# marc345/Dense2Sparse-ViT

Measured on AMD Instinct MI355X. Metric: training images/s, DeiT-S 224 keep_ratio=0.5 (dense-to-sparse ViT train step, teacher fwd + student fwd/bwd + AdamW), higher is better.
Workload: dtype f32; 1 GPU; DeiT-Small 224x224 patch16, 1-stage prune keep_ratio=0.5 @ block 3 (196->98 tokens), large LN predictor, kl_div mask loss, per-GPU batch 128; global_batch=128, parallelism=dp1

## Files before the change

dense2sparse-vit_amd/csrc/gemm_common.h:

```cpp
#pragma once
#include "d2s_common.h"

namespace d2s_gemm {

enum Epi : int {
    EPI_NONE = 0,
    EPI_BIAS = 1,
    EPI_BIAS_RELU = 2,
    EPI_BIAS_GELU = 3,
    EPI_BIAS_RESID = 4,
    EPI_MUL_GELU_GRAD = 5,
    EPI_MUL_RELU_MASK = 6,
    EPI_BIAS_ROWADD = 7,
    EPI_ACCUM = 8,
    EPI_BIAS_GELU_Z16 = 9,
    EPI_MUL_GELU_GRAD_Z16 = 10,
    EPI_BIAS_RESID_ROWSCALE = 11,
};

struct GemmArgs {
    const float* A; const float* B; float* C;
    const float* bias; const float* aux; float* aux_out;
    long lda, ldb, ldc, ldaux;
    int M, N, K;
    int epi;
    int k_per_slice;
    long slab_stride;
    int aux_rows;
    int vecA, vecB;
    int remap_rows_per_img; int remap_skip;
    int stagger;
    int vec_epilogue;
    float* colsum;
    int colsum_accumulate;
    const void* a16; void* c16;
    const void* b16;
    int aux_bf16;
    const float* rowscale; int rows_per_group;
};

typedef __bf16 bf16x4_epi __attribute__((ext_vector_type(4)));

template <int EPI, int MT, int NT>
__device__ __forceinline__ void store_tile_out(const GemmArgs& p, float* __restrict__ Cb, const f32x16 (&acc)[MT][NT], int mbase,
                                               int nbase, int half) {
#pragma unroll
    for (int nt = 0; nt < NT; ++nt) {
        const int n = nbase + nt * 32;
        if (n >= p.N) continue;
        float bias = 0.f;
        if (EPI == EPI_BIAS || EPI == EPI_BIAS_RELU || EPI == EPI_BIAS_GELU || EPI == EPI_BIAS_RESID || EPI == EPI_BIAS_ROWADD ||
            EPI == EPI_BIAS_RESID_ROWSCALE)
            bias = p.bias ? p.bias[n] : 0.f;
#pragma unroll
        for (int mt = 0; mt < MT; ++mt) {
#pragma unroll
            for (int r = 0; r < 16; ++r) {
                const int m = mbase + mt * 32 + mfma32_row(r, half);
                if (m >= p.M) continue;
                float v = acc[mt][nt][r];
                long orow = m;
                if (EPI == EPI_BIAS_ROWADD && p.remap_rows_per_img > 0)
                    orow = (long)m + (long)(m / p.remap_rows_per_img) * p.remap_skip + p.remap_skip;
                float* cp = Cb + orow * p.ldc + n;
                if (EPI == EPI_BIAS) v += bias;
                if (EPI == EPI_BIAS_RELU) v = fmaxf(v + bias, 0.f);
                if (EPI == EPI_BIAS_GELU) {
                    v += bias;
                    if (p.aux_out && p.aux_bf16) reinterpret_cast<__bf16*>(p.aux_out)[(long)m * p.ldc + n] = (__bf16)v;
                    else if (p.aux_out) p.aux_out[(long)m * p.ldc + n] = v;
                    v = gelu_erf(v);
                }
                if (EPI == EPI_BIAS_RESID) v += bias + p.aux[(long)m * p.ldaux + n];
                if (EPI == EPI_BIAS_RESID_ROWSCALE) {
                    const float s = p.rowscale[m / p.rows_per_group];
                    v = s == 0.f ? p.aux[(long)m * p.ldaux + n] : s * (v + bias) + p.aux[(long)m * p.ldaux + n];
                }
                if (EPI == EPI_MUL_GELU_GRAD)
                    v *= gelu_erf_grad(p.aux_bf16 ? (float)reinterpret_cast<const __bf16*>(p.aux)[(long)m * p.ldaux + n] : p.aux[(long)m * p.ldaux + n]);
                if (EPI == EPI_MUL_RELU_MASK) v = p.aux[(long)m * p.ldaux + n] > 0.f ? v : 0.f;
                if (EPI == EPI_BIAS_ROWADD) v += bias + p.aux[(long)(m % p.aux_rows) * p.ldaux + n];
                if (EPI == EPI_ACCUM) v += *cp;
                *cp = v;
            }
        }
    }
}

__host__ __device__ constexpr int epi_stage_floats(int NT) { return 16 * (NT * 32 + 4); }

template <int EPI, int MT, int NT, bool C16 = false>
// ... 125 lines not shown
```

dense2sparse-vit_amd/csrc/gemm_f32.hip:

```cpp
#include "gemm_common.h"

namespace {
using namespace d2s_gemm;

constexpr int BK = 16;

#ifdef D2S_STAMPS
__device__ unsigned long long g_stamps_f32[8 * 65536];
#define FSTAMP(i) if (threadIdx.x == 0 && blockIdx.x < 65536 && blockIdx.z == 0) g_stamps_f32[8 * blockIdx.x + (i)] = __builtin_amdgcn_s_memrealtime()
#define FSTAMPC(i) if (threadIdx.x == 0 && blockIdx.x < 65536 && blockIdx.z == 0) g_stamps_f32[8 * blockIdx.x + (i)] = __builtin_amdgcn_s_memtime()
#define FSTAMPID(i) if (threadIdx.x == 0 && blockIdx.x < 65536 && blockIdx.z == 0) g_stamps_f32[8 * blockIdx.x + (i)] = \
    ((unsigned long long)__builtin_amdgcn_s_getreg((15 << 11) | (0 << 6) | 4)) | ((unsigned long long)__builtin_amdgcn_s_getreg((3 << 11) | (0 << 6) | 20) << 32)
#else
#define FSTAMP(i)
#define FSTAMPC(i)
#define FSTAMPID(i)
#endif

template <int LAY, int BR>
__device__ __forceinline__ void load_tile(const float* __restrict__ P, long ld, int row0, int k0, int rows, int kend,
                                          int vec, int tid, f32x4 (&r)[BR / 64]) {
#pragma unroll
    for (int i = 0; i < BR / 64; ++i) {
        const int f = tid + i * 256;
// ... 196 lines not shown
        f32x4 t = csum[0];
#pragma unroll
        for (int i = 1; i < BM / 64; ++i) t += csum[i];
        *reinterpret_cast<f32x4*>(&smem[(tid / CH) * BM + (tid % CH) * 4]) = t;
        __syncthreads();
        if (tid < BM && row0 + tid < p.M) {
            float s = 0.f;
#pragma unroll
            for (int g = 0; g < G; ++g) s += smem[g * BM + tid];
            float* o = p.colsum + (long)blockIdx.z * p.M + row0 + tid;
            *o = (gridDim.z == 1 && p.colsum_accumulate) ? *o + s : s;
        }
        __syncthreads();
    }

    FSTAMP(2); FSTAMPC(5);
    float* Cb = p.C + (long)blockIdx.z * p.slab_stride;
    const int epi = (gridDim.z > 1) ? (int)EPI_NONE : p.epi;
    static_assert(4 * epi_stage_floats(NT) <= 2 * BK * (BM + BN), "epilogue staging must fit the operand buffers");
    if (p.vec_epilogue) {
        store_tile_dispatch_lds<MT, NT>(epi, p, Cb, acc, row0 + wm * WM, col0 + wn * WN, lane, smem + wave * epi_stage_floats(NT));
#ifdef D2S_STAMPS
        __builtin_amdgcn_s_waitcnt(0);
        FSTAMP(3);
#endif
        return;
    }
    const int mbase = row0 + wm * WM, nbase = col0 + wn * WN + l31;
    switch (epi) {
        case EPI_BIAS: store_tile_out<EPI_BIAS, MT, NT>(p, Cb, acc, mbase, nbase, half); break;
        case EPI_BIAS_RELU: store_tile_out<EPI_BIAS_RELU, MT, NT>(p, Cb, acc, mbase, nbase, half); break;
        case EPI_BIAS_GELU: store_tile_out<EPI_BIAS_GELU, MT, NT>(p, Cb, acc, mbase, nbase, half); break;
        case EPI_BIAS_RESID: store_tile_out<EPI_BIAS_RESID, MT, NT>(p, Cb, acc, mbase, nbase, half); break;
        case EPI_MUL_GELU_GRAD: store_tile_out<EPI_MUL_GELU_GRAD, MT, NT>(p, Cb, acc, mbase, nbase, half); break;
        case EPI_MUL_RELU_MASK: store_tile_out<EPI_MUL_RELU_MASK, MT, NT>(p, Cb, acc, mbase, nbase, half); break;
        case EPI_BIAS_ROWADD: store_tile_out<EPI_BIAS_ROWADD, MT, NT>(p, Cb, acc, mbase, nbase, half); break;
        case EPI_ACCUM: store_tile_out<EPI_ACCUM, MT, NT>(p, Cb, acc, mbase, nbase, half); break;
        case EPI_BIAS_RESID_ROWSCALE: store_tile_out<EPI_BIAS_RESID_ROWSCALE, MT, NT>(p, Cb, acc, mbase, nbase, half); break;
        default: store_tile_out<EPI_NONE, MT, NT>(p, Cb, acc, mbase, nbase, half); break;
    }
}

template <int BR>
__device__ __forceinline__ void store_tile_rk(float* __restrict__ S, int tid, const f32x4 (&r)[BR / 64]) {
#pragma unroll
    for (int i = 0; i < BR / 64; ++i) {
        const int f = tid + i * 256;
        const int row = f >> 2, kq = f & 3;
        *reinterpret_cast<f32x4*>(&S[row * BK + ((kq ^ ((row >> 2) & 3)) << 2)]) = r[i];
    }
}

template <int BLAY, int BM, int BN>
__global__ __launch_bounds__(256, (BM == 128 && BN == 128) ? 3 : 1) void gemm_f32_rk_kernel(GemmArgs p) {
    constexpr int WM = BM / 2, WN = BN / 2, MT = WM / 32, NT = WN / 32;
    __shared__ __attribute__((aligned(16))) float smem[2 * BK * (BM + BN)];
    float* As = smem;
    float* Bs = smem + 2 * BK * BM;
    const int tid = threadIdx.x, lane = tid & 63, wave = tid >> 6;
    const int half = lane >> 5, l31 = lane & 31;
    const int wm = wave >> 1, wn = wave & 1;
    const int nbm = (p.M + BM - 1) / BM, nbn = (p.N + BN - 1) / BN;
    const int nwg = nbm * nbn;
    int bid = blockIdx.x;
    {
        const int q = nwg >> 3, r = nwg & 7, xcd = bid & 7, idx = bid >> 3;
        bid = (xcd < r ? xcd * (q + 1) : r * (q + 1) + (xcd - r) * q) + idx;
    }
    const int bm = bid / nbn, bn = bid % nbn;
    const int row0 = bm * BM, col0 = bn * BN;
    const int kbeg = blockIdx.z * p.k_per_slice;
    const int kend = min(p.K, kbeg + p.k_per_slice);
    const int nk = (kend - kbeg + BK - 1) / BK;

    f32x16 acc[MT][NT];
#pragma unroll
    for (int i = 0; i < MT; ++i)
#pragma unroll
        for (int j = 0; j < NT; ++j)
#pragma unroll
            for (int r = 0; r < 16; ++r) acc[i][j][r] = 0.f;

    f32x4 ra[BM / 64], rb[BN / 64];
    long offa[BM / 64], offb[BN / 64];
    tile_offsets<0, BM>(p.lda, row0, p.M, tid, offa);
    tile_offsets<BLAY, BN>(p.ldb, col0, p.N, tid, offb);
    if (nk > 0) {
        load_tile_fast<0, BM>(p.A, p.lda, kbeg, offa, ra);
        load_tile_fast<BLAY, BN>(p.B, p.ldb, kbeg, offb, rb);
        store_tile_rk<BM>(As, tid, ra);
        if (BLAY == 0) store_tile_rk<BN>(Bs, tid, rb);
        else store_tile<1, BN>(Bs, tid, rb);
    }
    __syncthreads();

    int a_off[MT][2], b_off[NT][2];
#pragma unroll
    for (int i = 0; i < MT; ++i) {
        const int row = wm * WM + i * 32 + l31;
#pragma unroll
        for (int c = 0; c < 2; ++c) a_off[i][c] = row * BK + (((2 * half + c) ^ ((row >> 2) & 3)) << 2);
    }
#pragma unroll
    for (int j = 0; j < NT; ++j) {
        const int row = wn * WN + j * 32 + l31;
#pragma unroll
        for (int c = 0; c < 2; ++c) b_off[j][c] = row * BK + (((2 * half + c) ^ ((row >> 2) & 3)) << 2);
    }

    for (int kt = 0; kt < nk; ++kt) {
        const int cur = kt & 1;
        const int kn = kbeg + min(kt + 1, nk - 1) * BK;
        load_tile_fast<0, BM>(p.A, p.lda, kn, offa, ra);
        load_tile_fast<BLAY, BN>(p.B, p.ldb, kn, offb, rb);
        const float* Ac = As + cur * BK * BM;
        const float* Bc = Bs + cur * BK * BN;
        f32x4 av[MT][2], bv[NT][2];
#pragma unroll
        for (int c = 0; c < 2; ++c) {
#pragma unroll
            for (int i = 0; i < MT; ++i) av[i][c] = *reinterpret_cast<const f32x4*>(Ac + a_off[i][c]);
            if (BLAY == 0) {
#pragma unroll
                for (int j = 0; j < NT; ++j) bv[j][c] = *reinterpret_cast<const f32x4*>(Bc + b_off[j][c]);
            }
        }
#pragma unroll
        for (int s = 0; s < 8; ++s) {
            float bs[NT];
            if (BLAY == 0) {
#pragma unroll
                for (int j = 0; j < NT; ++j) bs[j] = bv[j][s >> 2][s & 3];
            } else {
                const int k = 8 * half + s;
                const int sw = (((k >> 2) & 3) << 3) ^ ((k & 1) << 4);
#pragma unroll
                for (int j = 0; j < NT; ++j) bs[j] = Bc[k * BN + ((wn * WN + j * 32 + l31) ^ sw)];
            }
#pragma unroll
            for (int i = 0; i < MT; ++i)
#pragma unroll
                for (int j = 0; j < NT; ++j) acc[i][j] = mfma32(av[i][s >> 2][s & 3], bs[j], acc[i][j]);
        }
        if (kt + 1 < nk) {
            store_tile_rk<BM>(As + (cur ^ 1) * BK * BM, tid, ra);
            if (BLAY == 0) store_tile_rk<BN>(Bs + (cur ^ 1) * BK * BN, tid, rb);
            else store_tile<1, BN>(Bs + (cur ^ 1) * BK * BN, tid, rb);
        }
        __syncthreads();
    }

    float* Cb = p.C + (long)blockIdx.z * p.slab_stride;
    const int epi = (gridDim.z > 1) ? (int)EPI_NONE : p.epi;
    store_tile_dispatch_lds<MT, NT>(epi, p, Cb, acc, row0 + wm * WM, col0 + wn * WN, lane, smem + wave * epi_stage_floats(NT));
}

__global__ __launch_bounds__(256) void splitk_reduce_kernel(const float* __restrict__ ws, float* __restrict__ C,
                                                            long ldc, int M, int N, int slabs, long slab_stride,
                                                            int accumulate, const float* __restrict__ colsum_ws,
                                                            float* __restrict__ colsum_out) {
    const long idx = (long)blockIdx.x * 256 + threadIdx.x;
    const long total = (long)M * N;
    if (idx >= total) {
        const long m = idx - total;
        if (colsum_out && m < M) {
            float s = 0.f;
            for (int z = 0; z < slabs; ++z) s += colsum_ws[(long)z * M + m];
            colsum_out[m] = accumulate ? colsum_out[m] + s : s;
        }
        return;
    }
    const int m = (int)(idx / N), n = (int)(idx % N);
    float s = 0.f;
    for (int z = 0; z < slabs; ++z) s += ws[(long)z * slab_stride + (long)m * N + n];
    float* cp = C + (long)m * ldc + n;
    *cp = accumulate ? (*cp + s) : s;
}

__global__ __launch_bounds__(256) void splitk_reduce_vec_kernel(const float* __restrict__ ws, float* __restrict__ C, long ldc, int M, int N,
                                                                int slabs, long slab_stride, int accumulate,
                                                                const float* __restrict__ colsum_ws, float* __restrict__ colsum_out) {
    const long idx = (long)blockIdx.x * 256 + threadIdx.x;
    const int nq = N >> 2;
    const long total = (long)M * nq;
    if (idx >= total) {
        const long m = idx - total;
        if (colsum_out && m < M) {
            float s = 0.f;
            for (int z = 0; z < slabs; ++z) s += colsum_ws[(long)z * M + m];
            colsum_out[m] = accumulate ? colsum_out[m] + s : s;
        }
        return;
    }
    const int m = (int)(idx / nq), n = (int)(idx % nq) * 4;
    const float* src = ws + (long)m * N + n;
    f32x4 s = {0.f, 0.f, 0.f, 0.f};
    for (int z = 0; z < slabs; ++z) {
        const f32x4 v = *reinterpret_cast<const f32x4*>(src + (long)z * slab_stride);
#pragma unroll
        for (int j = 0; j < 4; ++j) s[j] += v[j];
    }
    f32x4* cp = reinterpret_cast<f32x4*>(C + (long)m * ldc + n);
    if (accumulate) {
        const f32x4 o = *cp;
#pragma unroll
        for (int j = 0; j < 4; ++j) s[j] += o[j];
    }
// ... 88 lines not shown
#pragma unroll
    for (int i = 0; i < 4; ++i) {
        const int f = tid + i * 256, c = f >> 4, r4 = (f & 15) * 4;
        if (c0 + c < C) {
#pragma unroll
            for (int j = 0; j < 4; ++j)
                if (r0 + r4 + j < R) dst[(long)(c0 + c) * R + r0 + r4 + j] = t[r4 + j][c];
        }
    }
}

__global__ __launch_bounds__(256) void colsum_partial_kernel(const float* __restrict__ X, long ldx, int M, int N,
                                                             int rows_per_slice, float* __restrict__ part) {
    __shared__ float red[4][64];
    const int lane = threadIdx.x & 63, wave = threadIdx.x >> 6;
    const int n = blockIdx.x * 64 + lane;
    const int m0 = blockIdx.y * rows_per_slice, m1 = min(M, m0 + rows_per_slice);
    float s = 0.f;
    if (n < N)
        for (int m = m0 + wave; m < m1; m += 4) s += X[(long)m * ldx + n];
    red[wave][lane] = s;
    __syncthreads();
    if (wave == 0 && n < N) part[(long)blockIdx.y * N + n] = red[0][lane] + red[1][lane] + red[2][lane] + red[3][lane];
}
__global__ __launch_bounds__(1024) void colsum_fold_wide_kernel(const float* __restrict__ part, int N, int slices, float* __restrict__ out,
                                                                int accumulate) {
    __shared__ float red[64][17];
    const int col = threadIdx.x & 15, kl = threadIdx.x >> 4;
    const int n = blockIdx.x * 16 + col;
    float s = 0.f;
    if (n < N)
        for (int z = kl; z < slices; z += 64) s += part[(long)z * N + n];
    red[kl][col] = s;
    __syncthreads();
    if (kl == 0 && n < N) {
        float t = 0.f;
#pragma unroll 8
        for (int k = 0; k < 64; ++k) t += red[k][col];
        out[n] = accumulate ? out[n] + t : t;
    }
}

__global__ __launch_bounds__(256) void colsum_final_kernel(const float* __restrict__ part, int N, int slices,
                                                           float* __restrict__ out, int accumulate) {
    const int n = blockIdx.x * 256 + threadIdx.x;
    if (n >= N) return;
    float s = 0.f;
    for (int z = 0; z < slices; ++z) s += part[(long)z * N + n];
    out[n] = accumulate ? out[n] + s : s;
}


struct Tile { int bm, bn; float penalty; };
inline Tile pick_tile(int M, int N) {
    const Tile cand[4] = {{128, 128, 1.00f}, {128, 64, 1.04f}, {64, 128, 1.05f}, {64, 64, 1.10f}};
    Tile best = cand[0];
    float best_cost = 1e30f;
    for (const Tile& t : cand) {
        const long nwg = (long)((M + t.bm - 1) / t.bm) * ((N + t.bn - 1) / t.bn);
        const long per_cu = (nwg + 255) / 256;
        const float pipe = per_cu >= 3 ? 1.0f : per_cu == 2 ? 0.85f : 0.6f;
        const float cost = (float)per_cu * t.bm * t.bn * t.penalty / pipe;
        if (cost < best_cost) { best_cost = cost; best = t; }
    }
    return best;
}

template <int ALAY, int BLAY, bool FAST>
inline void launch_gemm_f(const Tile& t, dim3 grid, hipStream_t stream, const GemmArgs& p) {
    dim3 block(256);
    if (t.bm == 128 && t.bn == 128) hipLaunchKernelGGL((gemm_f32_kernel<ALAY, BLAY, 128, 128, FAST>), grid, block, 0, stream, p);
    else if (t.bm == 128) hipLaunchKernelGGL((gemm_f32_kernel<ALAY, BLAY, 128, 64, FAST>), grid, block, 0, stream, p);
    else if (t.bn == 128) hipLaunchKernelGGL((gemm_f32_kernel<ALAY, BLAY, 64, 128, FAST>), grid, block, 0, stream, p);
    else hipLaunchKernelGGL((gemm_f32_kernel<ALAY, BLAY, 64, 64, FAST>), grid, block, 0, stream, p);
}
template <int BLAY>
inline void launch_gemm_rk(const Tile& t, dim3 grid, hipStream_t stream, const GemmArgs& p) {
    dim3 block(256);
    if (t.bm == 128 && t.bn == 128) hipLaunchKernelGGL((gemm_f32_rk_kernel<BLAY, 128, 128>), grid, block, 0, stream, p);
    else if (t.bm == 128) hipLaunchKernelGGL((gemm_f32_rk_kernel<BLAY, 128, 64>), grid, block, 0, stream, p);
    else if (t.bn == 128) hipLaunchKernelGGL((gemm_f32_rk_kernel<BLAY, 64, 128>), grid, block, 0, stream, p);
    else hipLaunchKernelGGL((gemm_f32_rk_kernel<BLAY, 64, 64>), grid, block, 0, stream, p);
}
template <int ALAY, int BLAY>
inline void launch_gemm(const Tile& t, dim3 grid, hipStream_t stream, const GemmArgs& p, bool fast) {
    if (fast && p.vec_epilogue && ALAY == 0) launch_gemm_rk<BLAY>(t, grid, stream, p);
    else if (fast) launch_gemm_f<ALAY, BLAY, true>(t, grid, stream, p);
    else launch_gemm_f<ALAY, BLAY, false>(t, grid, stream, p);
}

}

namespace d2s_gemm {
size_t split_workspace_bytes(int split, int M, int N, int K);
int launch_split_gemm(const GemmArgs& p, int b_cols, int split, void* workspace, size_t workspace_bytes, hipStream_t stream);
size_t split_tn_pieces_bytes(int split, int M, int N, int K);
int split_tn_colsum_partials(int K);
bool split_tn_use_dma(int M, int N, int K);
int split_tn_dma_slices(int M, int N, int K);
int launch_split_gemm_tn(const GemmArgs& p, int split, int slices, void* pieces_ws, float* colsum_part, hipStream_t stream, int* colsum_parts);
}
static int splitk_target() {
    static const int t = [] {
        int dev = 0, cus = 0;
        if (hipGetDevice(&dev) != hipSuccess || hipDeviceGetAttribute(&cus, hipDeviceAttributeMultiprocessorCount, dev) != hipSuccess || cus <= 0)
            cus = 256;
        return 3 * cus;
    }();
    return t;
}
static inline size_t ws_align(size_t x) { return (x + 255) & ~(size_t)255; }
extern "C" size_t d2s_colsum_workspace_bytes(int M, int N);
extern "C" int d2s_colsum_f32(const float* X, long ldx, int M, int N, float* out, int accumulate, void* workspace,
                              size_t workspace_bytes, hipStream_t stream);
static int nt_slices(int tiles, int K) {
    if (K < 512 || tiles > 512) return 1;
    int best = 1;
    float best_cost = 1e30f;
    const int smax = K / 256 < 8 ? K / 256 : 8;
    for (int sl = 1; sl <= smax; ++sl) {
        const long per_cu = ((long)tiles * sl + 255) / 256;
        const float pipe = per_cu >= 3 ? 1.0f : per_cu == 2 ? 0.85f : 0.6f;
        const float cost = (float)per_cu / ((float)sl * pipe) + 0.04f * (sl - 1);
        if (cost < best_cost - 1e-6f) { best_cost = cost; best = sl; }
    }
    return best;
}
static int splitk_slices(int tiles, int K) {
    int slices = splitk_target() / tiles;
    const int max_slices = (K + 255) / 256;
    if (slices > max_slices) slices = max_slices;
    if (slices < 1) slices = 1;
    return slices;
}

#ifdef D2S_STAMPS
extern "C" int d2s_debug_read_stamps_f32(unsigned long long* host_out, int n_wg) {
    return hipMemcpyFromSymbol(host_out, HIP_SYMBOL(g_stamps_f32), (size_t)n_wg * 8 * sizeof(unsigned long long)) == hipSuccess ? 0 : -1;
}
#endif

extern "C" {

size_t d2s_gemm_f32_workspace_bytes(int layout, int M, int N, int K, int mode) {
    if (layout != 2 && mode != 0) return split_workspace_bytes(mode == 1 ? 3 : 1, M, N, K);
    if (layout != 2) {
        const Tile t = pick_tile(M, N);
        const int sl = nt_slices(((M + t.bm - 1) / t.bm) * ((N + t.bn - 1) / t.bn), K);
        return sl > 1 ? (size_t)sl * M * N * sizeof(float) : 0;
    }
    const int tiles = ((M + 127) / 128) * ((N + 127) / 128);
    if (mode != 2) {
        const int slices = splitk_slices(tiles, K);
        return slices <= 1 ? 0 : ((size_t)slices * M * N + (size_t)slices * M) * sizeof(float);
    }
    const int slices = split_tn_use_dma(M, N, K) ? split_tn_dma_slices(M, N, K) : splitk_slices(tiles, K);
    return ws_align(((size_t)(slices + 1) * M * N) * sizeof(float)) + ws_align(split_tn_pieces_bytes(1, M, N, K)) + (size_t)split_tn_colsum_partials(K) * M * sizeof(float);
}

static int gemm_impl(int layout, const float* A, long lda, const float* B, long ldb, float* C, long ldc, int M, int N,
                     int K, int epilogue, const float* bias, const float* aux, long ldaux, float* aux_out, int aux_rows,
                     int remap_rows_per_img, int remap_skip, int accumulate, void* workspace, size_t workspace_bytes,
                     hipStream_t stream, float* colsum_out, int mode, const void* a16 = nullptr, void* c16 = nullptr, const void* b16 = nullptr,
                     const float* rowscale = nullptr, int rows_per_group = 0) {
    if (b16 && (mode != 2 || (layout != 2 && (K % 32 != 0 || !aligned16(b16))) || (layout == 2 && (reinterpret_cast<uintptr_t>(b16) & 7)))) return D2S_ERR_ARG;
    if ((!A && !(a16 && layout != 2) && !(b16 && layout == 2)) || (!B && !(a16 && layout == 2) && !(b16 && layout != 2)) || (!C && !c16) || M <= 0 || N <= 0 || K <= 0 || layout < 0 || layout > 2 || mode < 0 || mode > 2) return D2S_ERR_ARG;
    if ((a16 || c16) && (mode != 2 || (layout != 2 && accumulate) || remap_rows_per_img > 0)) return D2S_ERR_ARG;
    if (layout == 2 && c16) return D2S_ERR_ARG;
    if (layout == 2 && a16) {
        if ((reinterpret_cast<uintptr_t>(a16) & 7) != 0) return D2S_ERR_ARG;
    }
    if ((a16 && layout != 2 && (K % 32 != 0 || !aligned16(a16))) || (c16 && (N % 32 != 0 || !aligned16(c16)))) return D2S_ERR_ARG;
    int aux_bf16 = 0;
    if (epilogue == EPI_BIAS_GELU_Z16 || epilogue == EPI_MUL_GELU_GRAD_Z16) {
        const float* z = epilogue == EPI_BIAS_GELU_Z16 ? aux_out : aux;
        if (mode != 2 || layout == 2 || !z || (reinterpret_cast<uintptr_t>(z) & 7) || N % 4 != 0 || (epilogue == EPI_MUL_GELU_GRAD_Z16 && ldaux % 4 != 0) ||
            (epilogue == EPI_BIAS_GELU_Z16 && ldc % 4 != 0))
            return D2S_ERR_ARG;
        aux_bf16 = 1;
        epilogue = epilogue == EPI_BIAS_GELU_Z16 ? EPI_BIAS_GELU : EPI_MUL_GELU_GRAD;
    }
    if (epilogue == EPI_BIAS_RESID_ROWSCALE) {
        if (!rowscale || rows_per_group <= 0 || layout == 2 || accumulate || !aux) return D2S_ERR_ARG;
    } else if (epilogue < EPI_NONE || epilogue > EPI_ACCUM) return D2S_ERR_ARG;
    if ((epilogue == EPI_BIAS_RESID || epilogue == EPI_MUL_GELU_GRAD || epilogue == EPI_MUL_RELU_MASK ||
         epilogue == EPI_BIAS_ROWADD) && !aux)
        return D2S_ERR_ARG;
    GemmArgs p;
    p.aux_bf16 = aux_bf16;
    p.A = A; p.B = B; p.C = C; p.bias = bias; p.aux = aux; p.aux_out = aux_out;
    p.lda = lda; p.ldb = ldb; p.ldc = ldc; p.ldaux = ldaux;
    p.M = M; p.N = N; p.K = K; p.epi = epilogue; p.aux_rows = aux_rows > 0 ? aux_rows : 1;
    p.remap_rows_per_img = remap_rows_per_img; p.remap_skip = remap_skip;
    p.colsum = nullptr; p.colsum_accumulate = accumulate;
    p.a16 = a16; p.c16 = c16; p.b16 = b16;
    p.rowscale = rowscale; p.rows_per_group = rows_per_group > 0 ? rows_per_group : 1;
    {
        p.stagger = 0;
        p.vec_epilogue = 0;
    }
    const int alay = layout == 2 ? 1 : 0, blay = layout == 0 ? 0 : 1;
    p.vecA = aligned16(A) && (lda % 4 == 0) && (alay == 0 ? (K % 4 == 0) : (M % 4 == 0));
    p.vecB = aligned16(B) && (ldb % 4 == 0) && (blay == 0 ? (K % 4 == 0) : (N % 4 == 0));
    if (mode != 0 && layout != 2) {
        if (accumulate) p.epi = EPI_ACCUM;
        p.k_per_slice = K;
        p.slab_stride = 0;
        return launch_split_gemm(p, layout == 1 ? 1 : 0, mode == 1 ? 3 : 1, workspace, workspace_bytes, stream);
    }
    if (layout == 2 && mode == 2) {
        const int tiles = ((M + 127) / 128) * ((N + 127) / 128);
        int slices = split_tn_use_dma(M, N, K) ? split_tn_dma_slices(M, N, K) : splitk_slices(tiles, K);
        const int Kp = ((K + 63) / 64) * 64;
        int kper = (((Kp + slices - 1) / slices + 63) / 64) * 64;
        slices = (Kp + kper - 1) / kper;
        const size_t slab_bytes = ws_align(((size_t)(slices + 1) * M * N) * sizeof(float));
        const size_t piece_bytes = ws_align(split_tn_pieces_bytes(1, M, N, K));
        const size_t cs_bytes = (size_t)split_tn_colsum_partials(K) * M * sizeof(float);
        if (!workspace || workspace_bytes < slab_bytes + piece_bytes + cs_bytes) return D2S_ERR_WORKSPACE;
        unsigned char* wsb = static_cast<unsigned char*>(workspace);
        p.k_per_slice = kper;
        p.epi = EPI_NONE;
        p.C = reinterpret_cast<float*>(wsb);
        p.ldc = N;
        p.slab_stride = (long)M * N;
        p.remap_rows_per_img = 0;
        float* cs_part = colsum_out ? reinterpret_cast<float*>(wsb + slab_bytes + piece_bytes) : nullptr;
        int cs_parts = 0;
        int rc = launch_split_gemm_tn(p, 1, slices, wsb + slab_bytes, cs_part, stream, &cs_parts);
        if (rc != D2S_OK) return rc;
        const long total = (long)M * N;
        hipLaunchKernelGGL(splitk_reduce_kernel, dim3((unsigned)((total + 255) / 256)), dim3(256), 0, stream,
                           reinterpret_cast<const float*>(wsb), C, ldc, M, N, slices, (long)M * N, accumulate,
                           static_cast<const float*>(nullptr), static_cast<float*>(nullptr));
        if (colsum_out)
            hipLaunchKernelGGL(colsum_fold_wide_kernel, dim3((M + 15) / 16), dim3(1024), 0, stream, cs_part, M, cs_parts,
                               colsum_out, accumulate);
        return d2s_check_launch();
    }
    Tile tile = layout == 2 ? Tile{128, 128, 1.f} : pick_tile(M, N);
    const int tiles = ((M + tile.bm - 1) / tile.bm) * ((N + tile.bn - 1) / tile.bn);
    int slices = layout == 2 ? splitk_slices(tiles, K) : nt_slices(tiles, K);
    int kper = (K + slices - 1) / slices;
    kper = ((kper + BK - 1) / BK) * BK;
    slices = (K + kper - 1) / kper;
    p.k_per_slice = kper;
    p.slab_stride = 0;
    float* realC = C;
    if (accumulate && layout != 2 && p.epi == EPI_NONE) p.epi = EPI_ACCUM;
    const GemmArgs real = p;
    if (slices > 1 && layout != 2) {
        const size_t need = (size_t)slices * M * N * sizeof(float);
        if (!workspace || workspace_bytes < need) return D2S_ERR_WORKSPACE;
        p.C = static_cast<float*>(workspace);
        p.ldc = N;
        p.slab_stride = (long)M * N;
        p.remap_rows_per_img = 0;
    } else if (slices > 1) {
        const size_t need = ((size_t)slices * M * N + (size_t)slices * M) * sizeof(float);
        if (!workspace || workspace_bytes < need) return D2S_ERR_WORKSPACE;
        p.C = static_cast<float*>(workspace);
        p.ldc = N;
        p.slab_stride = (long)M * N;
        p.remap_rows_per_img = 0;
        if (colsum_out) p.colsum = static_cast<float*>(workspace) + (size_t)slices * M * N;
    } else {
        if (accumulate) p.epi = EPI_ACCUM;
        p.colsum = colsum_out;
    }
    p.vec_epilogue = (epilogue_vec_ok(p) && (p.slab_stride % 4 == 0)) ? 1 : 0;
    dim3 grid(tiles, 1, slices), block(256);
    const bool fast = p.vecA && p.vecB && (K % BK == 0) && (alay == 0 || M >= 4) && (blay == 0 || N >= 4);
    if (layout == 0) launch_gemm<0, 0>(tile, grid, stream, p, fast);
    else if (layout == 1) launch_gemm<0, 1>(tile, grid, stream, p, fast);
    else launch_gemm<1, 1>(tile, grid, stream, p, fast);
    if (slices > 1 && layout != 2) {
        const long total = (long)M * N;
        hipLaunchKernelGGL(splitk_reduce_epi_kernel, dim3((unsigned)((total + 255) / 256)), block, 0, stream, real,
                           static_cast<const float*>(workspace), slices, (long)M * N);
    } else if (slices > 1) {
        if ((N % 4 == 0) && (ldc % 4 == 0) && aligned16(realC) && aligned16(workspace) && (((long)M * N) % 4 == 0)) {
            const long total = (long)M * (N / 4) + (colsum_out ? M : 0);
            hipLaunchKernelGGL(splitk_reduce_vec_kernel, dim3((unsigned)((total + 255) / 256)), block, 0, stream,
                               static_cast<const float*>(workspace), realC, ldc, M, N, slices, (long)M * N, accumulate, p.colsum, colsum_out);
        } else {
            const long total = (long)M * N + (colsum_out ? M : 0);
            hipLaunchKernelGGL(splitk_reduce_kernel, dim3((unsigned)((total + 255) / 256)), block, 0, stream,
                               static_cast<const float*>(workspace), realC, ldc, M, N, slices, (long)M * N, accumulate,
                               p.colsum, colsum_out);
        }
    }
    return d2s_check_launch();
}

int d2s_gemm_f32(int layout, const float* A, long lda, const float* B, long ldb, float* C, long ldc, int M, int N,
                 int K, int epilogue, const float* bias, const float* aux, long ldaux, float* aux_out, int aux_rows,
                 int remap_rows_per_img, int remap_skip, int accumulate, int mode, void* workspace, size_t workspace_bytes,
                 hipStream_t stream) {
    return gemm_impl(layout, A, lda, B, ldb, C, ldc, M, N, K, epilogue, bias, aux, ldaux, aux_out, aux_rows, remap_rows_per_img,
                     remap_skip, accumulate, workspace, workspace_bytes, stream, nullptr, mode);
}

int d2s_gemm_f32_bf16io(int layout, const float* A, long lda, const float* B, long ldb, float* C, long ldc, int M, int N, int K,
                        int epilogue, const float* bias, const float* aux, long ldaux, float* aux_out, const void* a_bf16, const void* b_bf16,
                        void* c_bf16, void* workspace, size_t workspace_bytes, hipStream_t stream) {
    if (layout == 2) return D2S_ERR_ARG;
    return gemm_impl(layout, A, lda, B, ldb, C, ldc, M, N, K, epilogue, bias, aux, ldaux, aux_out, 0, 0, 0, 0, workspace, workspace_bytes,
                     stream, nullptr, 2, a_bf16, c_bf16, b_bf16);
}

int d2s_gemm_f32_rowscale(int layout, const float* A, long lda, const float* B, long ldb, float* C, long ldc, int M, int N, int K,
                          const float* bias, const float* aux, long ldaux, const float* rowscale, int rows_per_group, int mode,
                          const void* a_bf16, const void* b_bf16, void* c_bf16, void* workspace, size_t workspace_bytes, hipStream_t stream) {
    if (layout == 2 || !rowscale || rows_per_group <= 0) return D2S_ERR_ARG;
    return gemm_impl(layout, A, lda, B, ldb, C, ldc, M, N, K, EPI_BIAS_RESID_ROWSCALE, bias, aux, ldaux, nullptr, 0, 0, 0, 0, workspace,
                     workspace_bytes, stream, nullptr, mode, a_bf16, c_bf16, b_bf16, rowscale, rows_per_group);
}

size_t d2s_linear_wgrad_workspace_bytes(int tokens, int n_out, int n_in, int mode) {
    return d2s_gemm_f32_workspace_bytes(2, n_out, n_in, tokens, mode);
}
int d2s_linear_wgrad_f32(const float* dy, long lddy, const float* x, long ldx, float* dW, long lddw, float* db, int tokens,
                         int n_out, int n_in, int accumulate, int mode, void* workspace, size_t workspace_bytes, hipStream_t stream) {
    return gemm_impl(2, dy, lddy, x, ldx, dW, lddw, n_out, n_in, tokens, EPI_NONE, nullptr, nullptr, 0, nullptr, 0, 0, 0,
                     accumulate, workspace, workspace_bytes, stream, db, mode);
}
int d2s_linear_wgrad_f32_bf16x(const float* dy, const void* dy_bf16, long lddy, const void* x_bf16, long ldx, float* dW, long lddw, float* db,
                               int tokens, int n_out, int n_in, int accumulate, void* workspace, size_t workspace_bytes, hipStream_t stream) {
    if (!x_bf16 || (!dy && !dy_bf16)) return D2S_ERR_ARG;
    return gemm_impl(2, dy, lddy, nullptr, ldx, dW, lddw, n_out, n_in, tokens, EPI_NONE, nullptr, nullptr, 0, nullptr, 0, 0, 0,
                     accumulate, workspace, workspace_bytes, stream, db, 2, x_bf16, nullptr, dy_bf16);
}

int d2s_transpose_f32(const float* src, float* dst, int R, int C, hipStream_t stream) {
    if (!src || !dst || R <= 0 || C <= 0) return D2S_ERR_ARG;
    hipLaunchKernelGGL(transpose_kernel, dim3((C + 63) / 64, (R + 63) / 64), dim3(256), 0, stream, src, dst, R, C);
    return d2s_check_launch();
}

int d2s_transpose_batched_f32(const float* src_base, float* dst_base, const void* tile_desc, int n_tiles, hipStream_t stream) {
    if (!src_base || !dst_base || !tile_desc || n_tiles <= 0) return D2S_ERR_ARG;
    static_assert(sizeof(TransposeTile) == 32, "descriptor layout is part of the C ABI");
    hipLaunchKernelGGL(transpose_batched_kernel, dim3(n_tiles), dim3(256), 0, stream, src_base, dst_base, static_cast<const TransposeTile*>(tile_desc));
    return d2s_check_launch();
}

size_t d2s_colsum_workspace_bytes(int M, int N) {
    int slices = (M + 511) / 512;
    if (slices > 128) slices = 128;
    if (slices < 1) slices = 1;
    return (size_t)slices * N * sizeof(float);
}

int d2s_colsum_f32(const float* X, long ldx, int M, int N, float* out, int accumulate, void* workspace,
                   size_t workspace_bytes, hipStream_t stream) {
// ... 15 lines not shown
```

dense2sparse-vit_amd/d2s/lib.py:

```python
import ctypes
import os

import torch

_HERE = os.path.dirname(os.path.abspath(__file__))
LIB_PATH = os.environ.get("D2S_LIB_PATH") or os.path.join(os.path.dirname(_HERE), "lib", "libd2s_hip.so")

P, I, L, F, Z = ctypes.c_void_p, ctypes.c_int, ctypes.c_long, ctypes.c_float, ctypes.c_size_t

_SIGS = {
    "d2s_gemm_f32_workspace_bytes": (Z, [I, I, I, I, I]),
    "d2s_gemm_f32": (I, [I, P, L, P, L, P, L, I, I, I, I, P, P, L, P, I, I, I, I, I, P, Z]),
    "d2s_gemm_f32_bf16io": (I, [I, P, L, P, L, P, L, I, I, I, I, P, P, L, P, P, P, P, P, Z]),
    "d2s_convert_bf16": (I, [P, P, L]),
    "d2s_linear_wgrad_workspace_bytes": (Z, [I, I, I, I]),
    "d2s_linear_wgrad_f32": (I, [P, L, P, L, P, L, P, I, I, I, I, I, P, Z]),
    "d2s_linear_wgrad_f32_bf16x": (I, [P, P, L, P, L, P, L, P, I, I, I, I, P, Z]),
    "d2s_batchnorm_workspace_bytes": (Z, [L, I]),
    "d2s_batchnorm_fwd": (I, [P, P, P, P, P, P, P, P, L, I, F, F, I, P, Z]),
    "d2s_batchnorm_bwd": (I, [P, P, P, P, P, P, P, P, I, I, I, L, I, P, Z]),
    "d2s_transpose_f32": (I, [P, P, I, I]),
    "d2s_transpose_batched_f32": (I, [P, P, P, I]),
    "d2s_colsum_workspace_bytes": (Z, [I, I]),
    "d2s_colsum_f32": (I, [P, L, I, I, P, I, P, Z]),
# ... 70 lines not shown
    "d2s_block_saved_floats": (L, [I, I, I, I, I, I]),
    "d2s_block_bwd_scratch_floats": (L, [I, I, I, I, I]),
    "d2s_block_workspace_bytes": (Z, [I, I, I, I, I]),
    "d2s_block_wgrad_workspace_bytes": (Z, [I, I, I, I, I]),
    "d2s_block_fwd_f32": (I, [P, P, I, I, I, I, I, F, F, P, P, P, I, I, P, Z]),
    "d2s_block_bwd_f32": (I, [P, P, P, P, P, I, I, I, I, I, F, P, P, P, I, P, Z, P, Z, P]),
    "d2s_drop_path_scales": (I, [P, P, I, I, ctypes.c_ulonglong]),
    "d2s_gemm_f32_rowscale": (I, [I, P, L, P, L, P, L, I, I, I, P, P, L, P, I, I, P, P, P, P, Z]),
    "d2s_scale_rows": (I, [P, P, P, L, I, I]),
    "d2s_drop_path_fwd": (I, [P, P, P, I, L]),
    "d2s_block_bwd_dp_scratch_floats": (L, [I, I, I, I, I]),
    "d2s_block_fwd_f32_dp": (I, [P, P, P, P, I, I, I, I, I, F, F, P, P, P, I, I, P, Z]),
    "d2s_block_bwd_f32_dp": (I, [P, P, P, P, P, P, P, I, I, I, I, I, F, P, P, P, I, P, Z, P, Z, P]),
    "d2s_adamw_chunk_elems": (I, None),
    "d2s_adamw_step": (I, [P, P, P, P, P, I, F, F, F, I, F, P]),
    "d2s_adamw_step_ema": (I, [P, P, P, P, P, I, F, F, F, I, F, P, P, F]),
    "d2s_adamw_step_clip": (I, [P, P, P, P, P, I, F, F, F, I, F, P, P, F, P]),
    "d2s_grad_accumulate": (I, [P, P, P, I, I]),
    "d2s_grad_clip_coef": (I, [P, P, I, F, F, P, P]),
    "d2s_augment_desc_ints": (I, None),
    "d2s_augment_images": (I, [P, L, P, I, I, I, I, I, I, ctypes.c_ulonglong, P, P]),
    "d2s_augment_labels": (I, [P, I, I, F, F, P]),
    "d2s_randaug_max_ops": (I, None),
    "d2s_randaug_op_ints": (I, None),
    "d2s_randaug_scratch_bytes": (Z, [I, I]),
    "d2s_randaug_apply": (I, [P, P, I, I, P, P]),
    "d2s_augment_ops_scratch_bytes": (Z, [I, I]),
    "d2s_augment_images_ops": (I, [P, L, P, P, I, I, I, I, I, I, ctypes.c_ulonglong, P, P, P]),
    "d2s_gumbel_noise": (I, [P, L, ctypes.c_ulonglong]),
    "d2s_gumbel_from_bits": (I, [P, P, L]),
    "d2s_gumbel_keep_fwd": (I, [P, P, P, P, P, P, P, L]),
    "d2s_gumbel_keep_bwd": (I, [P, P, P, P, P, P, L]),
    "d2s_policy_pool_fwd": (I, [P, P, P, P, P, I, I, I]),
    "d2s_policy_pool_bwd": (I, [P, P, P, P, P, P, P, P, I, I, I]),
    "d2s_ratio_rows_fwd": (I, [P, F, P, P, I, I]),
    "d2s_ratio_rows_bwd": (I, [P, P, F, P, I, I]),
}

_SIGS_EXT = {
    "d2s_attn_keyw_fwd_bf16": (I, [P, I, P, P, P, P, I, I, I, F]),
    "d2s_tome_match_bf16": (I, [P, I, I, I, I, P, P, P, P, P]),
}

_SIGS_SQUEEZE = {
    "d2s_squeeze_match": (I, [P, P, P, I, I, I, I, P, P]),
    "d2s_gather_squeeze_fwd": (I, [P, P, P, P, P, I, I, I, I, P, P]),
    "d2s_gather_squeeze_bwd": (I, [P, P, P, P, P, P, I, I, I, I, P]),
}

_SIGS_ATS = {
    "d2s_ats_select": (I, [P, P, I, P, P, I, I, I, I, I, I, P, P, P, P]),
}

_lib = None


class D2SError(RuntimeError):
    pass


def load():
    global _lib
    if _lib is not None:
        return _lib
    if not os.path.exists(LIB_PATH):
        raise D2SError(f"{LIB_PATH} not found - build it with `python -c 'import __graft_entry__ as g; g.build()'` "
                       "(or `make -C dense2sparse-vit_amd/csrc`). The d2s path has no CPU fallback.")
    lib = ctypes.CDLL(LIB_PATH)
    for name, (res, args) in list(_SIGS.items()) + list(_SIGS_EXT.items()) + list(_SIGS_SQUEEZE.items()) + list(_SIGS_ATS.items()):
        fn = getattr(lib, name)
        fn.restype = res
        fn.argtypes = [] if args is None else list(args) + ([P] if res is I else [])
    _lib = lib
    return lib


def exported_symbols():
    return sorted(_SIGS)


def extension_symbols():
    return sorted(_SIGS_EXT)


def squeeze_symbols():
    return sorted(_SIGS_SQUEEZE)


def ats_symbols():
    return sorted(_SIGS_ATS)


def ptr(t):
    if t is None:
        return None
    if not t.is_cuda:
        raise D2SError("d2s ops need device tensors (no CPU fallback)")
    return t.data_ptr()


_raw_stream = getattr(torch._C, "_cuda_getCurrentRawStream", None)
_cur_device = getattr(torch._C, "_cuda_getDevice", None)
_fns = {}


def stream():
    if _raw_stream is not None and _cur_device is not None:
        return _raw_stream(_cur_device())
    return torch.cuda.current_stream().cuda_stream


def _fn(name):
    f = _fns.get(name)
    if f is None:
        f = _fns[name] = getattr(load(), name)
    return f


def call(name, *args):
    rc = _fn(name)(*args, stream())
    if rc != 0:
        raise D2SError(f"{name} failed with code {rc}")


def query(name, *args):
    return _fn(name)(*args)
```

Baseline: 3591 images/s.

## Add mixed main/tail tile plans to f32 GEMM to balance the last wave

Lets the register-staged f32 GEMM kernel run a main region with 128-row tiles and a tail region with 64x64 tiles in a single launch. A planner sizes the main region from CU count and occupancy so the leftover tiles fill the last wave more evenly. Tile penalty weights now depend on B layout. Planned and forced-plan entry points are exported for testing. This adds extra template instantiations and a heuristic cost model that could choose worse plans for some shapes.

Result: no change. 3589 images/s (-0.1%).

```diff
diff --git a/dense2sparse-vit_amd/csrc/gemm_common.h b/dense2sparse-vit_amd/csrc/gemm_common.h
--- a/dense2sparse-vit_amd/csrc/gemm_common.h
+++ b/dense2sparse-vit_amd/csrc/gemm_common.h
@@ -37,6 +37,7 @@
     const void* b16;
     int aux_bf16;
     const float* rowscale; int rows_per_group;
+    int n_main; int tail_row0;
 };
 
 typedef __bf16 bf16x4_epi __attribute__((ext_vector_type(4)));
diff --git a/dense2sparse-vit_amd/csrc/gemm_f32.hip b/dense2sparse-vit_amd/csrc/gemm_f32.hip
--- a/dense2sparse-vit_amd/csrc/gemm_f32.hip
+++ b/dense2sparse-vit_amd/csrc/gemm_f32.hip
@@ -272,23 +272,22 @@
 }
 
 template <int BLAY, int BM, int BN>
-__global__ __launch_bounds__(256, (BM == 128 && BN == 128) ? 3 : 1) void gemm_f32_rk_kernel(GemmArgs p) {
+__device__ __forceinline__ void gemm_rk_tile(const GemmArgs& p, float* __restrict__ smem, int bid, int seg_row0, int seg_row_end) {
     constexpr int WM = BM / 2, WN = BN / 2, MT = WM / 32, NT = WN / 32;
-    __shared__ __attribute__((aligned(16))) float smem[2 * BK * (BM + BN)];
+    static_assert(4 * epi_stage_floats(NT) <= 2 * BK * (BM + BN), "epilogue staging must fit the operand buffers");
     float* As = smem;
     float* Bs = smem + 2 * BK * BM;
     const int tid = threadIdx.x, lane = tid & 63, wave = tid >> 6;
     const int half = lane >> 5, l31 = lane & 31;
     const int wm = wave >> 1, wn = wave & 1;
-    const int nbm = (p.M + BM - 1) / BM, nbn = (p.N + BN - 1) / BN;
+    const int nbm = (seg_row_end - seg_row0 + BM - 1) / BM, nbn = (p.N + BN - 1) / BN;
     const int nwg = nbm * nbn;
-    int bid = blockIdx.x;
     {
         const int q = nwg >> 3, r = nwg & 7, xcd = bid & 7, idx = bid >> 3;
         bid = (xcd < r ? xcd * (q + 1) : r * (q + 1) + (xcd - r) * q) + idx;
     }
     const int bm = bid / nbn, bn = bid % nbn;
-    const int row0 = bm * BM, col0 = bn * BN;
+    const int row0 = seg_row0 + bm * BM, col0 = bn * BN;
     const int kbeg = blockIdx.z * p.k_per_slice;
     const int kend = min(p.K, kbeg + p.k_per_slice);
     const int nk = (kend - kbeg + BK - 1) / BK;
@@ -373,6 +372,18 @@
     float* Cb = p.C + (long)blockIdx.z * p.slab_stride;
     const int epi = (gridDim.z > 1) ? (int)EPI_NONE : p.epi;
     store_tile_dispatch_lds<MT, NT>(epi, p, Cb, acc, row0 + wm * WM, col0 + wn * WN, lane, smem + wave * epi_stage_floats(NT));
+}
+
+template <int BLAY, int BM, int BN, int TBM = 0, int TBN = 0>
+__global__ __launch_bounds__(256, (BM == 128 && BN == 128) ? 3 : 1) void gemm_f32_rk_kernel(GemmArgs p) {
+    static_assert(TBM + TBN <= BM + BN, "the tail tile lives in a prefix of the main tile's LDS");
+    __shared__ __attribute__((aligned(16))) float smem[2 * BK * (BM + BN)];
+    if constexpr (TBM == 0) {
+        gemm_rk_tile<BLAY, BM, BN>(p, smem, blockIdx.x, 0, p.M);
+    } else {
+        if ((int)blockIdx.x < p.n_main) gemm_rk_tile<BLAY, BM, BN>(p, smem, blockIdx.x, 0, p.tail_row0);
+        else gemm_rk_tile<BLAY, TBM, TBN>(p, smem, (int)blockIdx.x - p.n_main, p.tail_row0, p.M);
+    }
 }
 
 __global__ __launch_bounds__(256) void splitk_reduce_kernel(const float* __restrict__ ws, float* __restrict__ C,
@@ -567,8 +578,8 @@
 
 
 struct Tile { int bm, bn; float penalty; };
-inline Tile pick_tile(int M, int N) {
-    const Tile cand[4] = {{128, 128, 1.00f}, {128, 64, 1.04f}, {64, 128, 1.05f}, {64, 64, 1.10f}};
+inline Tile pick_tile(int blay, int M, int N) {
+    const Tile cand[4] = {{128, 128, 1.00f}, {128, 64, blay == 0 ? 1.05f : 1.04f}, {64, 128, blay == 0 ? 1.04f : 1.05f}, {64, 64, 1.10f}};
     Tile best = cand[0];
     float best_cost = 1e30f;
     for (const Tile& t : cand) {
@@ -589,17 +600,93 @@
     else if (t.bn == 128) hipLaunchKernelGGL((gemm_f32_kernel<ALAY, BLAY, 64, 128, FAST>), grid, block, 0, stream, p);
     else hipLaunchKernelGGL((gemm_f32_kernel<ALAY, BLAY, 64, 64, FAST>), grid, block, 0, stream, p);
 }
+struct Plan { int bm, bn, tail_row0, tbm, tbn; };
+inline bool plan_has_tail(const Plan& pl, int M) { return pl.tbm > 0 && pl.tail_row0 < M; }
+inline Plan uniform_plan(const Tile& t, int M) { return Plan{t.bm, t.bn, (M + t.bm - 1) / t.bm * t.bm, 0, 0}; }
+
+inline int device_cus() {
+    static const int n = [] {
+        int dev = 0, cus = 0;
+        if (hipGetDevice(&dev) != hipSuccess || hipDeviceGetAttribute(&cus, hipDeviceAttributeMultiprocessorCount, dev) != hipSuccess || cus <= 0) {
+            (void)hipGetLastError();
+            cus = 256;
+        }
+        return cus;
+    }();
+    return n;
+}
+template <typename Kern>
+inline int residency_of(Kern kernel, int fallback) {
+    int n = 0;
+    if (hipOccupancyMaxActiveBlocksPerMultiprocessor(&n, kernel, 256, 0) != hipSuccess || n <= 0) {
+        (void)hipGetLastError();
+        return fallback;
+    }
+    return n;
+}
+inline int rk_residency(int blay, const Plan& pl, int M) {
+    static const int mixed[2][2] = {{residency_of(gemm_f32_rk_kernel<0, 128, 128, 64, 64>, 4), residency_of(gemm_f32_rk_kernel<0, 128, 64, 64, 64>, 6)},
+                                    {residency_of(gemm_f32_rk_kernel<1, 128, 128, 64, 64>, 4), residency_of(gemm_f32_rk_kernel<1, 128, 64, 64, 64>, 6)}};
+    static const int uni[2][4] = {{residency_of(gemm_f32_rk_kernel<0, 128, 128>, 4), residency_of(gemm_f32_rk_kernel<0, 128, 64>, 6),
+                                   residency_of(gemm_f32_rk_kernel<0, 64, 128>, 6), residency_of(gemm_f32_rk_kernel<0, 64, 64>, 8)},
+                                  {residency_of(gemm_f32_rk_kernel<1, 128, 128>, 4), residency_of(gemm_f32_rk_kernel<1, 128, 64>, 6),
+                                   residency_of(gemm_f32_rk_kernel<1, 64, 128>, 5), residency_of(gemm_f32_rk_kernel<1, 64, 64>, 8)}};
+    const int t = pl.bm == 128 ? (pl.bn == 128 ? 0 : 1) : (pl.bn == 128 ? 2 : 3);
+    return plan_has_tail(pl, M) ? mixed[blay][t] : uni[blay][t];
+}
+inline float tile_penalty(int bm, int bn) { return bm == 128 ? (bn == 128 ? 1.00f : 1.04f) : (bn == 128 ? 1.04f : 1.10f); }
+inline float segment_cost(long tiles, int cus, int resid, float tile_cost) {
+    const float per_cu = (float)tiles / (float)cus;
+    const long full = (long)(per_cu / resid);
+    const float x = (per_cu - (float)(full * resid)) / resid;
+    const float g = x <= 0.f ? 0.f : (0.2f + 1.1f * x < 1.f ? 0.2f + 1.1f * x : 1.f);
+    return ((float)full + g) * resid * tile_cost;
+}
+inline float plan_cost(const Plan& pl, int blay, int M, int N, int cus) {
+    const int resid = rk_residency(blay, pl, M);
+    const long nbn = (N + pl.bn - 1) / pl.bn;
+    if (!plan_has_tail(pl, M)) return segment_cost((long)((M + pl.bm - 1) / pl.bm) * nbn, cus, resid, pl.bm * pl.bn * tile_penalty(pl.bm, pl.bn));
+    const long tail_tiles = (long)((M - pl.tail_row0 + pl.tbm - 1) / pl.tbm) * ((N + pl.tbn - 1) / pl.tbn);
+    return segment_cost((long)(pl.tail_row0 / pl.bm) * nbn, cus, resid, pl.bm * pl.bn * tile_penalty(pl.bm, pl.bn)) +
+           segment_cost(tail_tiles, cus, resid, pl.tbm * pl.tbn * tile_penalty(pl.tbm, pl.tbn));
+}
+constexpr float TAIL_MARGIN = 0.96f;
+inline Plan plan_rk(int blay, int M, int N) {
+    const int cus = device_cus();
+    const Plan uni = uniform_plan(pick_tile(blay, M, N), M);
+    Plan best = uni;
+    if ((long)((M + uni.bm - 1) / uni.bm) * ((N + uni.bn - 1) / uni.bn) <= 512) return best;
+    float best_cost = plan_cost(uni, blay, M, N, cus) * TAIL_MARGIN;
+    Plan pl{128, 128, 0, 64, 64};
+    const long nbm = (M + 127) / 128, nbn = (N + 127) / 128;
+    if (nbm * nbn <= 512) return best;
+    const long group = (long)cus * rk_residency(blay, pl, M);
+    for (long g = nbm * nbn / group; g >= 1 && g + 1 >= nbm * nbn / group; --g) {
+        const long rows = g * group / nbn;
+        if (rows <= 0 || rows >= nbm) continue;
+        pl.tail_row0 = (int)rows * 128;
+        const float c = plan_cost(pl, blay, M, N, cus);
+        if (c < best_cost) { best_cost = c; best = pl; }
+    }
+    return best;
+}
+
 template <int BLAY>
-inline void launch_gemm_rk(const Tile& t, dim3 grid, hipStream_t stream, const GemmArgs& p) {
+inline void launch_gemm_rk(const Plan& t, int M, dim3 grid, hipStream_t stream, const GemmArgs& p) {
     dim3 block(256);
-    if (t.bm == 128 && t.bn == 128) hipLaunchKernelGGL((gemm_f32_rk_kernel<BLAY, 128, 128>), grid, block, 0, stream, p);
+    if (plan_has_tail(t, M)) {
+        if (t.bn == 128) hipLaunchKernelGGL((gemm_f32_rk_kernel<BLAY, 128, 128, 64, 64>), grid, block, 0, stream, p);
+        else hipLaunchKernelGGL((gemm_f32_rk_kernel<BLAY, 128, 64, 64, 64>), grid, block, 0, stream, p);
+    }
+    else if (t.bm == 128 && t.bn == 128) hipLaunchKernelGGL((gemm_f32_rk_kernel<BLAY, 128, 128>), grid, block, 0, stream, p);
     else if (t.bm == 128) hipLaunchKernelGGL((gemm_f32_rk_kernel<BLAY, 128, 64>), grid, block, 0, stream, p);
     else if (t.bn == 128) hipLaunchKernelGGL((gemm_f32_rk_kernel<BLAY, 64, 128>), grid, block, 0, stream, p);
     else hipLaunchKernelGGL((gemm_f32_rk_kernel<BLAY, 64, 64>), grid, block, 0, stream, p);
 }
 template <int ALAY, int BLAY>
-inline void launch_gemm(const Tile& t, dim3 grid, hipStream_t stream, const GemmArgs& p, bool fast) {
-    if (fast && p.vec_epilogue && ALAY == 0) launch_gemm_rk<BLAY>(t, grid, stream, p);
+inline void launch_gemm(const Plan& pl, dim3 grid, hipStream_t stream, const GemmArgs& p, bool fast) {
+    const Tile t{pl.bm, pl.bn, 1.f};
+    if (fast && p.vec_epilogue && ALAY == 0) launch_gemm_rk<BLAY>(pl, p.M, grid, stream, p);
     else if (fast) launch_gemm_f<ALAY, BLAY, true>(t, grid, stream, p);
     else launch_gemm_f<ALAY, BLAY, false>(t, grid, stream, p);
 }
@@ -616,13 +703,7 @@
 int launch_split_gemm_tn(const GemmArgs& p, int split, int slices, void* pieces_ws, float* colsum_part, hipStream_t stream, int* colsum_parts);
 }
 static int splitk_target() {
-    static const int t = [] {
-        int dev = 0, cus = 0;
-        if (hipGetDevice(&dev) != hipSuccess || hipDeviceGetAttribute(&cus, hipDeviceAttributeMultiprocessorCount, dev) != hipSuccess || cus <= 0)
-            cus = 256;
-        return 3 * cus;
-    }();
-    return t;
+    return 3 * device_cus();
 }
 static inline size_t ws_align(size_t x) { return (x + 255) & ~(size_t)255; }
 extern "C" size_t d2s_colsum_workspace_bytes(int M, int N);
@@ -660,7 +741,7 @@
 size_t d2s_gemm_f32_workspace_bytes(int layout, int M, int N, int K, int mode) {
     if (layout != 2 && mode != 0) return split_workspace_bytes(mode == 1 ? 3 : 1, M, N, K);
     if (layout != 2) {
-        const Tile t = pick_tile(M, N);
+        const Tile t = pick_tile(layout == 0 ? 0 : 1, M, N);
         const int sl = nt_slices(((M + t.bm - 1) / t.bm) * ((N + t.bn - 1) / t.bn), K);
         return sl > 1 ? (size_t)sl * M * N * sizeof(float) : 0;
     }
@@ -677,7 +758,16 @@
                      int K, int epilogue, const float* bias, const float* aux, long ldaux, float* aux_out, int aux_rows,
                      int remap_rows_per_img, int remap_skip, int accumulate, void* workspace, size_t workspace_bytes,
                      hipStream_t stream, float* colsum_out, int mode, const void* a16 = nullptr, void* c16 = nullptr, const void* b16 = nullptr,
-                     const float* rowscale = nullptr, int rows_per_group = 0) {
+                     const float* rowscale = nullptr, int rows_per_group = 0, const int* forced_plan = nullptr) {
+    Plan forced{0, 0, 0, 0, 0};
+    if (forced_plan) {
+        forced = Plan{forced_plan[0], forced_plan[1], forced_plan[2], forced_plan[3], forced_plan[4]};
+        if ((forced.bm != 64 && forced.bm != 128) || (forced.bn != 64 && forced.bn != 128) || forced.tail_row0 < 0) return D2S_ERR_ARG;
+        if (M > 0 && forced.tail_row0 < M &&
+            (forced.bm != 128 || forced.tbm != 64 || forced.tbn != 64 || forced.tail_row0 % forced.bm != 0 || layout == 2 || mode != 0))
+            return D2S_ERR_ARG;
+        if (forced.tail_row0 >= M) forced.tbm = forced.tbn = 0;
+    }
     if (b16 && (mode != 2 || (layout != 2 && (K % 32 != 0 || !aligned16(b16))) || (layout == 2 && (reinterpret_cast<uintptr_t>(b16) & 7)))) return D2S_ERR_ARG;
     if ((!A && !(a16 && layout != 2) && !(b16 && layout == 2)) || (!B && !(a16 && layout == 2) && !(b16 && layout != 2)) || (!C && !c16) || M <= 0 || N <= 0 || K <= 0 || layout < 0 || layout > 2 || mode < 0 || mode > 2) return D2S_ERR_ARG;
     if ((a16 || c16) && (mode != 2 || (layout != 2 && accumulate) || remap_rows_per_img > 0)) return D2S_ERR_ARG;
@@ -753,9 +843,10 @@
                                colsum_out, accumulate);
         return d2s_check_launch();
     }
-    Tile tile = layout == 2 ? Tile{128, 128, 1.f} : pick_tile(M, N);
-    const int tiles = ((M + tile.bm - 1) / tile.bm) * ((N + tile.bn - 1) / tile.bn);
+    Plan plan = layout == 2 ? uniform_plan(Tile{128, 128, 1.f}, M) : forced_plan ? forced : uniform_plan(pick_tile(blay, M, N), M);
+    int tiles = ((M + plan.bm - 1) / plan.bm) * ((N + plan.bn - 1) / plan.bn);
     int slices = layout == 2 ? splitk_slices(tiles, K) : nt_slices(tiles, K);
+    if (forced_plan && plan_has_tail(plan, M) && slices > 1) return D2S_ERR_ARG;
     int kper = (K + slices - 1) / slices;
     kper = ((kper + BK - 1) / BK) * BK;
     slices = (K + kper - 1) / kper;
@@ -784,11 +875,22 @@
         p.colsum = colsum_out;
     }
     p.vec_epilogue = (epilogue_vec_ok(p) && (p.slab_stride % 4 == 0)) ? 1 : 0;
+    const bool fast = p.vecA && p.vecB && (K % BK == 0) && (alay == 0 || M >= 4) && (blay == 0 || N >= 4);
+    const bool tail_ok = fast && p.vec_epilogue && alay == 0 && slices == 1;
+    if (forced_plan && plan_has_tail(plan, M) && !tail_ok) return D2S_ERR_ARG;
+    if (!forced_plan && tail_ok) plan = plan_rk(blay, M, N);
+    p.n_main = 0; p.tail_row0 = M;
+    if (plan_has_tail(plan, M)) {
+        p.tail_row0 = plan.tail_row0;
+        p.n_main = (plan.tail_row0 / plan.bm) * ((N + plan.bn - 1) / plan.bn);
+        tiles = p.n_main + ((M - plan.tail_row0 + plan.tbm - 1) / plan.tbm) * ((N + plan.tbn - 1) / plan.tbn);
+    } else {
+        tiles = ((M + plan.bm - 1) / plan.bm) * ((N + plan.bn - 1) / plan.bn);
+    }
     dim3 grid(tiles, 1, slices), block(256);
-    const bool fast = p.vecA && p.vecB && (K % BK == 0) && (alay == 0 || M >= 4) && (blay == 0 || N >= 4);
-    if (layout == 0) launch_gemm<0, 0>(tile, grid, stream, p, fast);
-    else if (layout == 1) launch_gemm<0, 1>(tile, grid, stream, p, fast);
-    else launch_gemm<1, 1>(tile, grid, stream, p, fast);
+    if (layout == 0) launch_gemm<0, 0>(plan, grid, stream, p, fast);
+    else if (layout == 1) launch_gemm<0, 1>(plan, grid, stream, p, fast);
+    else launch_gemm<1, 1>(plan, grid, stream, p, fast);
     if (slices > 1 && layout != 2) {
         const long total = (long)M * N;
         hipLaunchKernelGGL(splitk_reduce_epi_kernel, dim3((unsigned)((total + 255) / 256)), block, 0, stream, real,
@@ -816,6 +918,27 @@
                      remap_skip, accumulate, workspace, workspace_bytes, stream, nullptr, mode);
 }
 
+int d2s_gemm_f32_tile_plan(int layout, int M, int N, int K, int* plan) {
+    if (!plan || M <= 0 || N <= 0 || K <= 0 || layout < 0 || layout > 2) return D2S_ERR_ARG;
+    Plan pl = uniform_plan(layout == 2 ? Tile{128, 128, 1.f} : pick_tile(layout == 0 ? 0 : 1, M, N), M);
+    const int tiles = ((M + pl.bm - 1) / pl.bm) * ((N + pl.bn - 1) / pl.bn);
+    if (layout != 2 && K % BK == 0 && N % 4 == 0 && nt_slices(tiles, K) == 1) pl = plan_rk(layout == 0 ? 0 : 1, M, N);
+    plan[0] = pl.bm; plan[1] = pl.bn; plan[2] = pl.tail_row0; plan[3] = pl.tbm; plan[4] = pl.tbn;
+    return D2S_OK;
+}
+
+int d2s_gemm_f32_planned(int layout, const float* A, long lda, const float* B, long ldb, float* C, long ldc, int M, int N,
+                         int K, int epilogue, const float* bias, const float* aux, long ldaux, float* aux_out, int aux_rows,
+                         int remap_rows_per_img, int remap_skip, int accumulate, int mode, void* workspace, size_t workspace_bytes,
+                         int bm, int bn, int tail_row0, int tbm, int tbn, const float* rowscale, int rows_per_group, hipStream_t stream) {
+    const int plan[5] = {bm, bn, tail_row0, tbm, tbn};
+    if (epilogue == EPI_BIAS_RESID_ROWSCALE && (!rowscale || rows_per_group <= 0)) return D2S_ERR_ARG;
+    if (epilogue != EPI_BIAS_RESID_ROWSCALE && rowscale) return D2S_ERR_ARG;
+    return gemm_impl(layout, A, lda, B, ldb, C, ldc, M, N, K, epilogue, bias, aux, ldaux, aux_out, aux_rows, remap_rows_per_img,
+                     remap_skip, accumulate, workspace, workspace_bytes, stream, nullptr, mode, nullptr, nullptr, nullptr, rowscale,
+                     rows_per_group, plan);
+}
+
 int d2s_gemm_f32_bf16io(int layout, const float* A, long lda, const float* B, long ldb, float* C, long ldc, int M, int N, int K,
                         int epilogue, const float* bias, const float* aux, long ldaux, float* aux_out, const void* a_bf16, const void* b_bf16,
                         void* c_bf16, void* workspace, size_t workspace_bytes, hipStream_t stream) {
diff --git a/dense2sparse-vit_amd/d2s/lib.py b/dense2sparse-vit_amd/d2s/lib.py
--- a/dense2sparse-vit_amd/d2s/lib.py
+++ b/dense2sparse-vit_amd/d2s/lib.py
@@ -146,6 +146,12 @@
     "d2s_ats_select": (I, [P, P, I, P, P, I, I, I, I, I, I, P, P, P, P]),
 }
 
+_SIGS_GEMM = {
+    "d2s_gemm_f32_tile_plan": (I, [I, I, I, I, P]),
+    "d2s_gemm_f32_planned": (I, [I, P, L, P, L, P, L, I, I, I, I, P, P, L, P, I, I, I, I, I, P, Z, I, I, I, I, I, P, I]),
+}
+_NO_STREAM = {"d2s_gemm_f32_tile_plan"}
+
 _lib = None
 
 
@@ -161,10 +167,10 @@
         raise D2SError(f"{LIB_PATH} not found - build it with `python -c 'import __graft_entry__ as g; g.build()'` "
                        "(or `make -C dense2sparse-vit_amd/csrc`). The d2s path has no CPU fallback.")
     lib = ctypes.CDLL(LIB_PATH)
-    for name, (res, args) in list(_SIGS.items()) + list(_SIGS_EXT.items()) + list(_SIGS_SQUEEZE.items()) + list(_SIGS_ATS.items()):
+    for name, (res, args) in list(_SIGS.items()) + list(_SIGS_EXT.items()) + list(_SIGS_SQUEEZE.items()) + list(_SIGS_ATS.items()) + list(_SIGS_GEMM.items()):
         fn = getattr(lib, name)
         fn.restype = res
-        fn.argtypes = [] if args is None else list(args) + ([P] if res is I else [])
+        fn.argtypes = [] if args is None else list(args) + ([P] if res is I and name not in _NO_STREAM else [])
     _lib = lib
     return lib
 
@@ -183,6 +189,18 @@
 
 def ats_symbols():
     return sorted(_SIGS_ATS)
+
+
+def gemm_plan_symbols():
+    return sorted(_SIGS_GEMM)
+
+
+def gemm_tile_plan(layout, M, N, K):
+    plan = (ctypes.c_int * 5)()
+    rc = query("d2s_gemm_f32_tile_plan", layout, M, N, K, ctypes.addressof(plan))
+    if rc != 0:
+        raise D2SError(f"d2s_gemm_f32_tile_plan failed with code {rc}")
+    return tuple(plan)
 
 
 def ptr(t):
diff --git a/include/d2s_hip_gemm.h b/include/d2s_hip_gemm.h
--- /dev/null
+++ b/include/d2s_hip_gemm.h
@@ -0,0 +1,21 @@
+#ifndef D2S_HIP_GEMM_H
+#define D2S_HIP_GEMM_H
+
+#include "d2s_hip.h"
+
+#ifdef __cplusplus
+extern "C" {
+#endif
+
+int d2s_gemm_f32_tile_plan(int layout, int M, int N, int K, int* plan);
+
+int d2s_gemm_f32_planned(int layout, const float* A, long lda, const float* B, long ldb, float* C, long ldc, int M, int N, int K,
+                         int epilogue, const float* bias, const float* aux, long ldaux, float* aux_out, int aux_rows,
+                         int remap_rows_per_img, int remap_skip, int accumulate, int mode, void* workspace, size_t workspace_bytes,
+                         int bm, int bn, int tail_row0, int tbm, int tbn, const float* rowscale, int rows_per_group, d2s_stream_t stream);
+
+#ifdef __cplusplus
+}
+#endif
+
+#endif
```
